# kerry-he/fsae-mpc

Measured on AMD Instinct MI355X. Metric: QP solves/sec (batched LTV-MPC, N=40 nx=5 nu=2 fp64), higher is better.
Workload: dtype f64

## Files before the change

### fsae-mpc_amd/csrc/qp_solver.hip

```cpp
#include <hip/hip_runtime.h>
#include <math.h>
#include <stdint.h>
#include <stdlib.h>
#include <stdio.h>
#include "qp_solver.h"

typedef double v4d __attribute__((ext_vector_type(4)));
typedef double v2d __attribute__((ext_vector_type(2)));

#define DEVINL __device__ __forceinline__
#ifndef QP_SOLVE_REFINE_STEPS
#define QP_SOLVE_REFINE_STEPS 1
#endif
#ifndef QP_FULL_BARRIERS
#define WAVE_SYNC() do { __builtin_amdgcn_fence(__ATOMIC_SEQ_CST, "wavefront"); __builtin_amdgcn_wave_barrier(); } while (0)
#else
#define WAVE_SYNC() __syncthreads()
#endif

namespace {

DEVINL double rl(double v, int src) {
  int lo = __builtin_amdgcn_readlane(__double2loint(v), src);
  int hi = __builtin_amdgcn_readlane(__double2hiint(v), src);
// ... 310 lines not shown
  for (int o = 1; o < NBIN; o <<= 1) {
    const int a = tid >= o ? scan[tid - o] : 0;
    __syncthreads();
    scan[tid] += a;
    __syncthreads();
  }
  int run = scan[tid] - v;
  for (int ww = 0; ww < NWV; ++ww) { const int c = cnt[ww][tid]; cnt[ww][tid] = run; run += c; }
  __syncthreads();
  if (w < NWV)
    for (int i0 = lo; i0 < hi; i0 += 512) {
      int kv[8];
#pragma unroll
      for (int r = 0; r < 8; ++r) { const int i = i0 + 64 * r + lane; kv[r] = i < hi ? bin(i) : -1; }
#pragma unroll
      for (int r = 0; r < 8; ++r) {
        const bool on = kv[r] >= 0; const int k = on ? kv[r] : 0;
        int rank, size; group(k, on, rank, size);
        int base = on ? cnt[w][k] : 0;
        if (on) order[base + rank] = i0 + 64 * r + lane;
        if (on && rank == 0) cnt[w][k] = base + size;
      }
    }
}

#endif

struct Ctx {
  int n, m, T, Kq, J, JB, JT, np, ld, lane, c, q, nc, nb, ntr;
  const int* perm; const int* tcs; const int* aoff; const int* tend;
  const double* Aw; const double* Hw; const double* Ab; const double* Hb;
  double* rows;
  double* ring;
  double* cof;
  int rowlen;
  double* Ms;
  double* vec;
};
enum VecArr { V_X = 0, V_G, V_HX, V_R1, V_R2, V_P1, V_P2, V_P3, V_DX, V_E, V_NARR };

DEVINL double* rowp(const Ctx& k, int arr) { return k.rows + (size_t)arr * k.rowlen; }
DEVINL double* vecp(const Ctx& k, int arr) { return k.vec + arr * k.np; }

DEVINL bool row_valid(const Ctx& k, int js) {
  if (js < k.J) { const int s = 16 * js + k.c; return s < k.Kq && 4 * s + k.q < k.m; }
  return (js - k.J) * 64 + k.lane < k.n;
}

template <int T> DEVINL void hx_tiles(const Ctx& k, const double* X, double* HX) {
  double hx[T], hn[T][4], hc[T][4];
#pragma unroll
  for (int t = 0; t < T; ++t) hx[t] = 0.0;
#pragma unroll
  for (int Jt = 0; Jt < T; ++Jt)
#pragma unroll
    for (int p = 0; p < 4; ++p) hn[Jt][p] = k.Hw[((size_t)Jt * 4 + p) * 64 + k.lane];
#pragma unroll 1
  for (int I = 0; I < T; ++I) {
#pragma unroll
    for (int Jt = 0; Jt < T; ++Jt)
#pragma unroll
      for (int p = 0; p < 4; ++p) hc[Jt][p] = hn[Jt][p];
    if (I + 1 < T) {
#pragma unroll
      for (int Jt = 0; Jt < T; ++Jt)
#pragma unroll
// ... 31 lines not shown
#pragma unroll
  for (int I = 0; I < T; ++I) {
    xc[I] = XV[16 * I + k.c]; sc[I] = 0.0;
#pragma unroll
    for (int p = 0; p < 4; ++p) { xr[I][p] = XV[16 * I + k.q + 4 * p]; sr[I][p] = 0.0; }
  }
#pragma unroll
  for (int I = 0; I < T; ++I)
#pragma unroll
    for (int J = I; J < T; ++J) {
      const v4d& h = acc[Tri<T>::idx(I, J)];
#pragma unroll
      for (int p = 0; p < 4; ++p) {
        sc[J] = fma(h[p], xr[I][p], sc[J]);
        if (J > I) sr[I][p] = fma(h[p], xc[J], sr[I][p]);
      }
    }
  WAVE_SYNC();
#pragma unroll
  for (int J = 0; J < T; ++J) { const double v = q_sum(sc[J]); if (k.q == 0) HX[16 * J + k.c] = v; }
  WAVE_SYNC();
#pragma unroll
  for (int I = 0; I < T - 1; ++I)
#pragma unroll
    for (int p = 0; p < 4; ++p) { const double v = grp16_sum(sr[I][p]); if (k.c == 0) HX[16 * I + k.q + 4 * p] += v; }
}

template <int C> struct IC { static constexpr int value = C; };

#ifdef QP_DRAIN_STREAM
template <int T> struct StreamCfg {
  static constexpr int R = 3 * T;
};
template <int T> struct Stream {
  static constexpr int R = StreamCfg<T>::R;
  const char* gnext;
  int half;
  DEVINL void issue(const Ctx& k, int slot) {
    __builtin_amdgcn_global_load_lds((const __attribute__((address_space(1))) void*)(gnext + k.lane * 16),
                                     (__attribute__((address_space(3))) void*)(k.ring + slot * 128), 16, 0, 0);
    gnext += 1024;
  }
  DEVINL void start(const Ctx& k, int c0) {
    gnext = reinterpret_cast<const char*>(k.Aw); half = 0;
#pragma unroll
    for (int t = 0; t < T; ++t) if (t < c0) issue(k, t);
  }
  template <int C> DEVINL void next_pair(const Ctx& k, v2d* b, int cn) {
    asm volatile("s_waitcnt vmcnt(0)" ::: "memory");
    const int other = (half ^ 1) * T;
#pragma unroll
    for (int t = 0; t < T; ++t) if (t < cn) issue(k, other + t);
    asm volatile("" ::: "memory");
#pragma unroll
    for (int t = 0; t < C; ++t) b[t] = *reinterpret_cast<const v2d*>(k.ring + (half * T + t) * 128 + k.lane * 2);
    half ^= 1;
  }
  DEVINL void drain() { asm volatile("s_waitcnt vmcnt(0)" ::: "memory"); }
};
#else
template <int T> struct StreamCfg {
  static constexpr int D = 2 * T;
  static constexpr int R = D + T;
};
template <int T> struct Stream {
  static constexpr int D = StreamCfg<T>::D, R = StreamCfg<T>::R;
  const char* gnext; int slot_i, slot_e;
  DEVINL void issue(const Ctx& k) {
    __builtin_amdgcn_global_load_lds((const __attribute__((address_space(1))) void*)(gnext + k.lane * 16),
                                     (__attribute__((address_space(3))) void*)(k.ring + slot_i * 128), 16, 0, 0);
    gnext += 1024;
    slot_i = slot_i + 1 == R ? 0 : slot_i + 1;
  }
  DEVINL void start(const Ctx& k, int) {
    gnext = reinterpret_cast<const char*>(k.Aw); slot_i = 0; slot_e = 0;
#pragma unroll
    for (int j = 0; j < D; ++j) issue(k);
  }
  template <int C> DEVINL void next_pair(const Ctx& k, v2d* b, int) {
#pragma unroll
    for (int t = 0; t < C; ++t) issue(k);
    asm volatile("s_waitcnt vmcnt(%0)" :: "n"(D) : "memory");
#pragma unroll
    for (int t = 0; t < C; ++t) {
      int sl = slot_e + t; if (sl >= R) sl -= R;
      b[t] = *reinterpret_cast<const v2d*>(k.ring + sl * 128 + k.lane * 2);
    }
    slot_e += C; if (slot_e >= R) slot_e -= R;
  }
  DEVINL void drain() { asm volatile("s_waitcnt vmcnt(0)" ::: "memory"); }
};
#endif

template <int NA> struct CoefStage {
  double reg[NA > 0 ? NA : 1];
  DEVINL void load(const Ctx& k, const double* const* arr, int js) {
    const int jc = js < k.J ? js : k.J - 1;
#pragma unroll
    for (int a = 0; a < NA; ++a) reg[a] = arr[a][jc * 64 + k.lane];
  }
  DEVINL void commit(const Ctx& k) {
#pragma unroll
    for (int a = 0; a < NA; ++a) k.cof[a * 64 + k.lane] = reg[a];
  }
  DEVINL void read_pair(const Ctx& k, int s, v2d* out) const {
#pragma unroll
    for (int a = 0; a < NA; ++a) out[a] = *reinterpret_cast<const v2d*>(k.cof + a * 64 + k.q * 16 + (s & 15));
  }
};

template <int T, int NB> DEVINL void pass_syrk(const Ctx& k, v4d* acc, double* P1, double* P2, double* P3, double* MB) {
  constexpr int NBB = NB > 0 ? NB : 1;
  constexpr int NA = 4 + NB;
  const int JS = k.J * 64;
  const double* arr[NA];
  arr[0] = rowp(k, R_D); arr[1] = rowp(k, R_W1); arr[2] = rowp(k, R_W2); arr[3] = rowp(k, R_W3);
#pragma unroll
  for (int e = 0; e < NB; ++e) arr[4 + e] = k.Ab + (size_t)e * JS;
  double p1[T], p2[T], p3[T];
  double pb[NBB][T], sbb[NBB][NBB], pwb[3][NBB];
#pragma unroll
  for (int t = 0; t < T; ++t) { p1[t] = 0; p2[t] = 0; p3[t] = 0; }
#pragma unroll
  for (int e = 0; e < NBB; ++e) {
#pragma unroll
    for (int t = 0; t < T; ++t) pb[e][t] = 0;
#pragma unroll
    for (int f = 0; f < NBB; ++f) sbb[e][f] = 0;
    pwb[0][e] = pwb[1][e] = pwb[2][e] = 0;
  }
  Stream<T> st;
  CoefStage<NA> cs;
  int tr = 0;
  if (k.ntr > 0) { st.start(k, k.tcs[0]); cs.load(k, arr, 0); }
  auto phase = [&](auto Cc) __attribute__((always_inline)) {
    constexpr int C = decltype(Cc)::value;
    const int tr_end = k.tend[C];
    for (; tr < tr_end; ++tr) {
      if ((tr & 3) == 0) { cs.commit(k); cs.load(k, arr, (tr >> 2) + 1); }
#pragma unroll
      for (int u = 0; u < 2; ++u) {
        v2d b[C], cf[NA];
        st.template next_pair<C>(k, b, u == 0 ? C : (tr + 1 < tr_end ? C : (tr + 1 < k.ntr ? k.tcs[tr + 1] : 0)));
        cs.read_pair(k, 4 * tr + 2 * u, cf);
        asm volatile("" ::: "memory");
#pragma unroll
        for (int h = 0; h < 2; ++h) {
          double a[C], ab[NBB];
          const double dd = cf[0][h], w1 = cf[1][h], w2 = cf[2][h], w3 = cf[3][h];
#pragma unroll
          for (int e = 0; e < NB; ++e) ab[e] = cf[4 + e][h];
#pragma unroll
          for (int t = 0; t < C; ++t) a[t] = dd * b[t][h];
#pragma unroll
          for (int I = 0; I < C; ++I)
#pragma unroll
            for (int Jt = I; Jt < C; ++Jt)
              acc[Tri<T>::idx(I, Jt)] = __builtin_amdgcn_mfma_f64_16x16x4f64(a[I], b[Jt][h], acc[Tri<T>::idx(I, Jt)], 0, 0, 0);
#pragma unroll
          for (int t = 0; t < C; ++t) {
            p1[t] = fma(w1, b[t][h], p1[t]); p2[t] = fma(w2, b[t][h], p2[t]); p3[t] = fma(w3, b[t][h], p3[t]);
          }
#pragma unroll
          for (int e = 0; e < NB; ++e) {
// ... 6 lines not shown
          }
        }
      }
    }
  };
  if constexpr (T >= 1) phase(IC<1>{});
  if constexpr (T >= 2) phase(IC<2>{});
  if constexpr (T >= 3) phase(IC<3>{});
  if constexpr (T >= 4) phase(IC<4>{});
  if constexpr (T >= 5) phase(IC<5>{});
  if constexpr (T >= 6) phase(IC<6>{});
  if constexpr (T >= 7) phase(IC<7>{});
  if constexpr (T >= 8) phase(IC<8>{});
  if (k.ntr > 0) st.drain();
#pragma unroll
  for (int t = 0; t < T; ++t) {
    double v1 = q_sum(p1[t]), v2 = q_sum(p2[t]), v3 = q_sum(p3[t]);
    if (k.q == 0) { P1[16 * t + k.c] = v1; P2[16 * t + k.c] = v2; P3[16 * t + k.c] = v3; }
  }
#pragma unroll
  for (int e = 0; e < NB; ++e) {
#pragma unroll
    for (int t = 0; t < T; ++t) { const double vb = q_sum(pb[e][t]); if (k.q == 0) MB[e * k.np + 16 * t + k.c] = vb; }
    const double v1 = q_sum(pwb[0][e]), v2 = q_sum(pwb[1][e]), v3 = q_sum(pwb[2][e]);
    if (k.lane == 0) { P1[k.nc + e] = v1; P2[k.nc + e] = v2; P3[k.nc + e] = v3; }
#pragma unroll
    for (int f = 0; f < NB; ++f) {
      const double sv = q_sum(f >= e ? sbb[e][f] : sbb[f][e]);
      if (k.lane == 0) MB[e * k.np + k.nc + f] = sv;
    }
  }
}

template <int T, int NB, int NVEC, int FUSE> DEVINL void pass_Av(const Ctx& k, const double* const* vin, double* const* rout, double* Pcor, double* Pcor2 = nullptr, const double* const* cfarr = nullptr) {
  constexpr int NBB = NB > 0 ? NB : 1;
  constexpr int NC = FUSE == 1 ? 6 : (FUSE >= 2 ? 3 : 0);
  constexpr int NA = NC + NB;
  const int JS = k.J * 64;
  const double* arr[NA > 0 ? NA : 1];
  if (FUSE == 1) { arr[0] = rowp(k, R_RPL); arr[1] = rowp(k, R_CB1); arr[2] = rowp(k, R_CC1); arr[3] = rowp(k, R_RPU); arr[4] = rowp(k, R_CB2); arr[5] = rowp(k, R_CC2); }
  if (FUSE >= 2) { arr[0] = cfarr ? cfarr[0] : rowp(k, R_CB1); arr[1] = cfarr ? cfarr[1] : rowp(k, R_RPL); arr[2] = cfarr ? cfarr[2] : rowp(k, R_CC1); }
#pragma unroll
  for (int f = 0; f < NB; ++f) arr[NC + f] = k.Ab + (size_t)f * JS;
  double v[NVEC][T], vb[NVEC][NBB], pc[T], pcb[NBB], pd[FUSE >= 2 ? T : 1], pdb[NBB];
#pragma unroll
  for (int e = 0; e < NVEC; ++e) {
#pragma unroll
    for (int t = 0; t < T; ++t) v[e][t] = vin[e][16 * t + k.c];
#pragma unroll
    for (int f = 0; f < NB; ++f) vb[e][f] = vin[e][k.nc + f];
  }
#pragma unroll
  for (int t = 0; t < T; ++t) pc[t] = 0.0;
#pragma unroll
  for (int f = 0; f < NBB; ++f) { pcb[f] = 0.0; pdb[f] = 0.0; }
#pragma unroll
  for (int t = 0; t < (FUSE >= 2 ? T : 1); ++t) pd[t] = 0.0;
  double keep[NVEC + 1];
#pragma unroll
  for (int e = 0; e < NVEC + 1; ++e) keep[e] = 0.0;
  Stream<T> st;
  CoefStage<NA> cs;
  int tr = 0;
  if (k.ntr > 0) { st.start(k, k.tcs[0]); if (NA > 0) cs.load(k, arr, 0); }
  auto phase = [&](auto Cc) __attribute__((always_inline)) {
    constexpr int C = decltype(Cc)::value;
    const int tr_end = k.tend[C];
    for (; tr < tr_end; ++tr) {
      if (NA > 0 && (tr & 3) == 0) { cs.commit(k); cs.load(k, arr, (tr >> 2) + 1); }
#pragma unroll
      for (int u = 0; u < 2; ++u) {
        v2d b[C], cf[NA > 0 ? NA : 1];
        st.template next_pair<C>(k, b, u == 0 ? C : (tr + 1 < tr_end ? C : (tr + 1 < k.ntr ? k.tcs[tr + 1] : 0)));
        if (NA > 0) cs.read_pair(k, 4 * tr + 2 * u, cf);
        asm volatile("" ::: "memory");
#pragma unroll
        for (int h = 0; h < 2; ++h) {
          const int s = 4 * tr + 2 * u + h;
          const int cc = s & 15;
#pragma unroll
          for (int e = 0; e < NVEC; ++e) {
            double dsum = 0.0;
#pragma unroll
            for (int t = 0; t < C; ++t) dsum = fma(b[t][h], v[e][t], dsum);
            dsum = grp16_sum(dsum);
#pragma unroll
            for (int f = 0; f < NB; ++f) dsum = fma(cf[NC + f][h], vb[e][f], dsum);
            if (k.c == cc) keep[e] = dsum;
            if (FUSE >= 2 && e == 0) {
              const double pen = cf[0][h] * (dsum - cf[1][h]);
              const double ynew = cf[2][h] - pen;
              if (k.c == cc) keep[NVEC] = ynew;
#pragma unroll
              for (int t = 0; t < C; ++t) { pc[t] = fma(ynew, b[t][h], pc[t]); pd[t] = fma(pen, b[t][h], pd[t]); }
// ... 300 lines not shown
      rh[K][p] = v;
    }
}
template <int T, int NS> DEVINL void rhs_store(const Ctx& k, const v4d* rh, double* const* vecs) {
#pragma unroll
  for (int K = 0; K < T; ++K)
#pragma unroll
    for (int p = 0; p < 4; ++p) {
      const int i = 16 * K + k.q + 4 * p;
#pragma unroll
      for (int e = 0; e < NS; ++e) if (k.c == e) vecs[e][i] = rh[K][p];
    }
}

#ifndef QP_STAMPS
#define QP_STAMPS 0
#endif
#if QP_STAMPS
#define STAMP_DECL unsigned long long st_acc[16]; for (int i_ = 0; i_ < 16; ++i_) st_acc[i_] = 0; unsigned long long st_t0 = __builtin_amdgcn_s_memtime();
#define STAMP(id) do { __builtin_amdgcn_sched_barrier(0); unsigned long long t_ = __builtin_amdgcn_s_memtime(); st_acc[id] += t_ - st_t0; st_t0 = t_; __builtin_amdgcn_sched_barrier(0); } while (0)
#define STAMP_OUT do { if (P.dump && P.dump_stage == 9 && lane == 0) for (int i_ = 0; i_ < 16; ++i_) P.dump[(size_t)b * 16 + i_] = (double)st_acc[i_]; } while (0)
#else
#define STAMP_DECL
#define STAMP(id) do { } while (0)
#define STAMP_OUT do { } while (0)
#endif

#ifndef QP_REFINE_ATTEMPTS
#define QP_REFINE_ATTEMPTS 3
#endif
#ifndef QP_WAVES_PER_SIMD
#define QP_WAVES_PER_SIMD 1
#endif
template <int T, int NB> __global__ __launch_bounds__(64, QP_WAVES_PER_SIMD) void qp_solve_kernel(QpParams P) {
  const int b = P.order ? P.order[blockIdx.x] : blockIdx.x;
  Ctx k;
  const QpDims& d = P.d;
  k.n = d.n; k.m = d.m; k.T = T; k.Kq = d.Kq; k.J = d.J; k.JB = d.JB; k.JT = d.J + d.JB; k.np = d.np; k.ld = 0;
  k.lane = threadIdx.x; k.c = k.lane & 15; k.q = k.lane >> 4; k.nc = d.nc; k.nb = d.nb;
  double* ws = P.ws + (size_t)b * d.ws_per_qp;
  k.Aw = ws + d.off_Aw; k.Hw = ws + d.off_Hw; k.Ab = ws + d.off_Ab; k.Hb = ws + d.off_Hb;
  k.rows = ws + d.off_rows; k.rowlen = d.rowlen; k.ntr = d.ntr;
  k.perm = reinterpret_cast<const int*>(ws + d.off_meta); k.tcs = k.perm + (size_t)(d.J > 0 ? d.J : 1) * 64;
  k.aoff = k.tcs + d.ntr; k.tend = k.aoff + d.ntr + 1;
  extern __shared__ double lds[];
  k.Ms = nullptr; k.vec = lds;
  double* MB = lds + (size_t)V_NARR * d.np;
  double* YL = MB + (size_t)(NB > 0 ? NB : 1) * d.np;
  k.ring = YL + T * 272;
  k.cof = k.ring + StreamCfg<T>::R * 128;
  double* SCR = k.ring;
  const double* gw = ws + d.off_gw;
  const double* Es = ws + d.off_E;
  const double* Fs = ws + d.off_F;
  const int lane = k.lane, n = k.n, JT = k.JT, J = k.J, nc = k.nc, nb = k.nb;
  constexpr int NT = Tri<T>::NT;
  constexpr int NBB = NB > 0 ? NB : 1;

#define X vecp(k, V_X)
#define G vecp(k, V_G)
#define HX vecp(k, V_HX)
#define R1 vecp(k, V_R1)
#define R2 vecp(k, V_R2)
#define P1 vecp(k, V_P1)
#define P2 vecp(k, V_P2)
#define P3 vecp(k, V_P3)
#define DX vecp(k, V_DX)
#define EV vecp(k, V_E)
#define aL rowp(k, R_L)
#define aU rowp(k, R_U)
#define aTL rowp(k, R_TL)
#define aTU rowp(k, R_TU)
#define aZL rowp(k, R_ZL)
#define aZU rowp(k, R_ZU)
#define aV rowp(k, R_V)
#define aD rowp(k, R_D)
#define aW1 rowp(k, R_W1)
#define aW2 rowp(k, R_W2)
#define aW3 rowp(k, R_W3)
#define aVA rowp(k, R_VA)
#define aVC rowp(k, R_VC)
#define aRPL rowp(k, R_RPL)
// ... 28 lines not shown
    double l = aL[ix], u = aU[ix];
    if (valid) {
      if (l > -INFINITY && u < INFINITY) {
        if (l > u) infeas = 1;
        if (!(u > l)) {
          const double eps = 1e-9 * fmax(1.0, fabs(l));
          l -= eps; u += eps; aL[ix] = l; aU[ix] = u;
        }
      }
      cnt_local += (l > -INFINITY) + (u < INFINITY);
    }
    if (js >= J) {
      const int i = (js - J) * 64 + lane;
      if (i < k.np) {
        double xi = 0.0;
        if (P.x_init) { const int ui = i < k.n ? qp_user_index(d, i) : -1; if (ui >= 0) { const double xs = P.x_init[(size_t)b * d.nu + ui] / EV[i]; if (fabs(xs) < INFINITY) xi = xs; } }
        if (valid) { if (l > -INFINITY && xi < l) xi = l; if (u < INFINITY && xi > u) xi = u; }
        X[i] = xi;
      }
    }
  }
  const double cnt = fmax(1.0, wave_sum((double)cnt_local));
  infeas = wave_max((double)infeas) > 0;
  WAVE_SYNC();

  STAMP_DECL
  int flag = 1, it = 0, flag_polished = 0;
  double fval_s = 0.0, merit_s = INFINITY;
  if (infeas) { flag = -2; }
  if (ws[d.off_bad] != 0.0) flag = -1;

  {
    const double* vin[1] = {X}; double* rout[1] = {aV};
    pass_Av<T, NB, 1, 0>(k, vin, rout, nullptr);
    for (int jb = 0; jb < k.JB; ++jb) { const int i = jb * 64 + lane; aV[(J + jb) * 64 + lane] = i < n ? X[i] : 0.0; }
  }
  const double T0 = 10.0, Z0 = 100.0;
  for (int js = 0; js < JT; ++js) {
    const int ix = js * 64 + lane;
    const bool valid = row_valid(k, js);
    const double l = aL[ix], u = aU[ix], v = aV[ix];
    const bool hl = valid && l > -INFINITY, hu = valid && u < INFINITY;
    aTL[ix] = hl ? fmax(v - l, T0) : 1.0;
    aTU[ix] = hu ? fmax(u - v, T0) : 1.0;
    aZL[ix] = hl ? Z0 : 0.0;
    aZU[ix] = hu ? Z0 : 0.0;
    aW3[ix] = (js < J) ? ((hl ? Z0 : 0.0) - (hu ? Z0 : 0.0)) : 0.0;
  }
  WAVE_SYNC();
  {
    hx_full(X);
    pass_Atw<T, NB>(k, aW3, P3);
    WAVE_SYNC();
    for (int jb = 0; jb < k.JB; ++jb) {
      const int i = jb * 64 + lane, ix = (J + jb) * 64 + lane;
      if (i < n) {
        const double r = HX[i] + G[i] - P3[i];
        if (aL[ix] > -INFINITY) aZL[ix] = fmax(r, 0.0) + Z0;
        if (aU[ix] < INFINITY) aZU[ix] = fmax(-r, 0.0) + Z0;
      }
    }
    WAVE_SYNC();
  }

  double saved_merit = INFINITY, best_res = INFINITY;
  int have_saved = 0, stall = 0;
  double* XS = ws + d.off_save;
  double* LAMS = ws + d.off_save + k.np;

  auto row1_body = [&](int ix, bool valid, double l, double u, double v, double tl, double tu, double zl, double zu,
                       double& s_gap, double& m_rp) {
    const bool hl = valid && l > -INFINITY, hu = valid && u < INFINITY;
    const double rpl = hl ? v - l - tl : 0.0, rpu = hu ? u - v - tu : 0.0;
    const double dl_ = hl ? zl / tl : 0.0, du_ = hu ? zu / tu : 0.0;
    aRPL[ix] = rpl; aRPU[ix] = rpu;
    rowp(k, R_CB1)[ix] = dl_; rowp(k, R_CC1)[ix] = hl ? dl_ / tl : 0.0;
    rowp(k, R_CB2)[ix] = du_; rowp(k, R_CC2)[ix] = hu ? du_ / tu : 0.0;
    aD[ix] = dl_ + du_;
    aW1[ix] = -dl_ * rpl + du_ * rpu;
    aW2[ix] = (hl ? 1.0 / tl : 0.0) - (hu ? 1.0 / tu : 0.0);
    aW3[ix] = (hl ? zl : 0.0) - (hu ? zu : 0.0);
    s_gap += (hl ? tl * zl : 0.0) + (hu ? tu * zu : 0.0);
    const double sc = fmax(1.0, fabs(v));
    if (hl) m_rp = fmax(m_rp, fabs(rpl) / fmax(sc, fabs(l)));
    if (hu) m_rp = fmax(m_rp, fabs(rpu) / fmax(sc, fabs(u)));
  };
  struct Slot { int ix; bool valid; double l, u, v, tl, tu, zl, zu, va, vc, w2, rpl, rpu; };
  auto load_slot = [&](int js) {
    Slot s_;
    const int jc = js < JT ? js : JT - 1;
    s_.ix = jc * 64 + lane; s_.valid = js < JT && row_valid(k, jc);
    const int ix = s_.ix;
    s_.l = aL[ix]; s_.u = aU[ix]; s_.v = aV[ix]; s_.tl = aTL[ix]; s_.tu = aTU[ix]; s_.zl = aZL[ix]; s_.zu = aZU[ix];
    s_.va = aVA[ix]; s_.vc = aVC[ix]; s_.w2 = aW2[ix]; s_.rpl = aRPL[ix]; s_.rpu = aRPU[ix];
    return s_;
  };
  double gap = 0.0, rp_rel = 0.0;

  v4d acc[NT];
  v4d rh[T];
  double Ubb[NBB][NBB];
  auto border_solve = [&](double* R) __attribute__((always_inline)) {
    if (NB > 0) {
      double yb[NBB], xb[NBB];
#pragma unroll
      for (int e = 0; e < NB; ++e) {
        double dsum = 0.0;
        for (int h = 0; h < 2; ++h) { const int i = lane + 64 * h; if (i < nc) dsum = fma(MB[e * k.np + i], R[i], dsum); }
        double tt = R[nc + e] - wave_sum(dsum);
#pragma unroll
        for (int g2 = 0; g2 < e; ++g2) tt -= Ubb[g2][e] * yb[g2];
        yb[e] = tt / Ubb[e][e];
      }
#pragma unroll
      for (int e = NB - 1; e >= 0; --e) {
        double tt = yb[e];
#pragma unroll
        for (int f = e + 1; f < NB; ++f) tt -= Ubb[e][f] * xb[f];
        xb[e] = tt / Ubb[e][e];
      }
      WAVE_SYNC();
      for (int h = 0; h < 2; ++h) {
        const int i = lane + 64 * h;
        if (i < nc) {
          double r = R[i];
#pragma unroll
          for (int e = 0; e < NB; ++e) r = fma(-MB[e * k.np + i], xb[e], r);
          R[i] = r;
// ... 132 lines not shown
  };
  auto solve1 = [&](double* V) __attribute__((always_inline)) {
#ifdef QP_MFMA_SOLVES
    const double* vin[1] = {V}; double* vout[1] = {V};
    rhs_load<T, 1>(k, rh, vin);
    reg_forward<T>(k, acc, YL, rh);
    if (NB > 0) {
      rhs_store<T, 1>(k, rh, vout);
      WAVE_SYNC();
      border_solve(V);
      rhs_load<T, 1>(k, rh, vin);
    }
    reg_backward<T>(k, acc, YL, rh, SCR);
    rhs_store<T, 1>(k, rh, vout);
#else
    double yv[T][4];
    vec_forward<T, false>(k, acc, YL, V, yv);
    if (NB > 0) {
      WAVE_SYNC();
      vec_rows_store<T>(k, yv, V);
      WAVE_SYNC();
      border_solve(V);
      vec_rows_load<T>(k, V, yv);
    }
    WAVE_SYNC();
    vec_backward<T, false>(k, acc, YL, yv, V);
#endif
  };

  STAMP(0);
  for (it = 0; flag == 1; ++it) {
    if (it == 0) {
      double s_gap = 0, m_rp = 0;
      for (int js = 0; js < JT; ++js) {
        const int ix = js * 64 + lane;
        row1_body(ix, row_valid(k, js), aL[ix], aU[ix], aV[ix], aTL[ix], aTU[ix], aZL[ix], aZU[ix], s_gap, m_rp);
      }
      gap = wave_sum(s_gap);
      rp_rel = wave_max(m_rp);
      WAVE_SYNC();
    }
    const double mu = gap / cnt;

    STAMP(1);
#ifdef QP_HX_SEPARATE
    hx_full(X);
    STAMP(2);
    acc_init<T>(k, acc);
#else
    acc_init<T>(k, acc);
    hx_from_acc<T>(k, acc, X, HX);
    hx_border(X);
    STAMP(2);
#endif
    pass_syrk<T, NB>(k, acc, P1, P2, P3, MB);
    WAVE_SYNC();
    STAMP(3);
    double fl = 0, m_rd = 0;
    for (int h = 0; h < 2; ++h) {
      const int i = lane + 64 * h;
      if (i < n) {
        const int ix = (J + (i >> 6)) * 64 + (i & 63);
        const double gz = P3[i] + aW3[ix];
        fl += 0.5 * X[i] * HX[i] + G[i] * X[i];
        const double sc = fmax(1.0, fmax(fabs(G[i]), fmax(fabs(HX[i]), fabs(gz))));
        m_rd = fmax(m_rd, fabs(HX[i] + G[i] - gz) / sc);
      }
    }
    const double fval = wave_sum(fl);
    const double rd_rel = wave_max(m_rd);
    const double gap_rel = gap / fmax(1.0, fabs(fval));
    const double merit = (fabs(fval) < INFINITY && fabs(gap_rel) < INFINITY) ? fmax(rd_rel, fmax(rp_rel, gap_rel)) : INFINITY;
    fval_s = fval; merit_s = merit;
    const bool res_ok = merit <= P.tol;
#ifdef QP_DEBUG_DUMP
    if (P.dump && P.dump_stage == 5 && b == P.dump_iter && lane == 0 && it < 120) {
      double* o_ = P.dump + 16 * it;
      o_[0] = merit; o_[1] = rd_rel; o_[2] = rp_rel; o_[3] = gap_rel; o_[4] = mu; o_[5] = fval; o_[6] = (double)have_saved; o_[7] = saved_merit;
    }
#endif
    if (!(merit < INFINITY)) { flag = have_saved ? 2 : -1; break; }
    if (merit <= P.tol_loose && merit < saved_merit) {
      for (int i = lane; i < k.np; i += 64) XS[i] = X[i];
      for (int js = 0; js < JT; ++js) LAMS[js * 64 + lane] = aW3[js * 64 + lane];
      have_saved = 1; saved_merit = merit;
    } else if (merit > P.tol_loose && rp_rel <= P.tol_loose && gap_rel <= P.tol_loose) {
      double dgap = 0, m_rd2 = 0, lamfix[2] = {0.0, 0.0};
      for (int h = 0; h < 2; ++h) {
// ... 53 lines not shown
    }
    if (it >= P.max_iter) { flag = have_saved ? 2 : 1; break; }

    {
      const double* vin[2] = {R1, R2}; double* rout[2] = {aVA, aVC};
      pass_Av<T, NB, 2, 1>(k, vin, rout, P1);
      for (int jb = 0; jb < k.JB; ++jb) {
        const int i = jb * 64 + lane;
        aVA[(J + jb) * 64 + lane] = i < n ? R1[i] : 0.0;
        aVC[(J + jb) * 64 + lane] = i < n ? R2[i] : 0.0;
      }
    }
    STAMP(7);
    double a_aff = 1.0, s1 = 0.0, s2 = 0.0;
    auto row2_body = [&](const Slot& r, int js) {
      const bool hl = r.valid && r.l > -INFINITY, hu = r.valid && r.u < INFINITY;
      double w = 0.0;
      if (hl) {
        const double dt = r.va + r.rpl, dz = -r.zl - (r.zl / r.tl) * dt;
        if (dt < 0) a_aff = fmin(a_aff, -r.tl / dt);
        if (dz < 0) a_aff = fmin(a_aff, -r.zl / dz);
        s1 += r.tl * dz + r.zl * dt; s2 += dt * dz;
        w -= dt * dz / r.tl;
      }
      if (hu) {
        const double dt = -r.va + r.rpu, dz = -r.zu - (r.zu / r.tu) * dt;
        if (dt < 0) a_aff = fmin(a_aff, -r.tu / dt);
        if (dz < 0) a_aff = fmin(a_aff, -r.zu / dz);
        s1 += r.tu * dz + r.zu * dt; s2 += dt * dz;
        w += dt * dz / r.tu;
      }
      if (js >= J && js < JT) aW1[r.ix] = w;
    };
    for (int js = 0; js < JT; js += 2) {
      const Slot r0 = load_slot(js), r1 = load_slot(js + 1);
      row2_body(r0, js); row2_body(r1, js + 1);
    }
    a_aff = wave_min(a_aff);
    s1 = wave_sum(s1); s2 = wave_sum(s2);
    const double mu_aff = fmax(0.0, gap + a_aff * (s1 + a_aff * s2)) / cnt;
    double sigma = mu > 0 ? (mu_aff / mu) * (mu_aff / mu) * (mu_aff / mu) : 0.0;
    if (sigma > 1.0) sigma = 1.0;
    {
      const double mu_floor = 1e-5 * P.tol * fmax(1.0, fabs(fval)) / cnt;
      if (mu > 0 && sigma < mu_floor / mu) sigma = fmin(1.0, mu_floor / mu);
    }
    const double smu = sigma * mu;
    const double cw = a_aff >= 0.05 ? 1.0 : 0.0;
    WAVE_SYNC();
    STAMP(8);
    if (cw != 0.0) {
    STAMP(9);
    for (int h = 0; h < 2; ++h) {
      const int i = lane + 64 * h;
      if (i < k.np) { const int ix = (J + (i >> 6)) * 64 + (i & 63); DX[i] = i < n ? P1[i] + aW1[ix] : 0.0; }
    }
    WAVE_SYNC();
    solve1(DX);
    WAVE_SYNC();
    STAMP(10);
    {
      const double* vin[1] = {DX}; double* rout[1] = {aW2};
      pass_Av<T, NB, 1, 0>(k, vin, rout, nullptr);
      for (int jb = 0; jb < k.JB; ++jb) { const int i = jb * 64 + lane; aW2[(J + jb) * 64 + lane] = i < n ? DX[i] : 0.0; }
    }
    STAMP(11);
    } else {
      for (int i = lane; i < k.np; i += 64) DX[i] = 0.0;
      for (int js = 0; js < JT; ++js) aW2[js * 64 + lane] = 0.0;
      WAVE_SYNC();
    }
    for (int h = 0; h < 2; ++h) {
      const int i = lane + 64 * h;
      if (i < n) DX[i] = R1[i] + smu * R2[i] + DX[i];
    }
    double amax = 1e300, bp = 0, bdp = 0, bd = 0, bdd = 0, q1 = 0.0, q2 = 0.0;
    auto row3a_body = [&](const Slot& r, int js) {
      const bool hl = r.valid && r.l > -INFINITY, hu = r.valid && r.u < INFINITY;
      const double dv = r.va + smu * r.vc + r.w2;
      if (js < JT) aVC[r.ix] = dv;
      if (hl) {
        const double dta = r.va + r.rpl, dza = -r.zl - (r.zl / r.tl) * dta;
        const double cl = smu - cw * dta * dza;
        const double dt = dv + r.rpl, dz = -r.zl + cl / r.tl - (r.zl / r.tl) * dt;
        if (dt < 0 && -r.tl / dt < amax) { amax = -r.tl / dt; bp = r.tl; bdp = dt; bd = r.zl; bdd = dz; }
        if (dz < 0 && -r.zl / dz < amax) { amax = -r.zl / dz; bp = r.zl; bdp = dz; bd = r.tl; bdd = dt; }
        q1 += r.tl * dz + r.zl * dt; q2 += dt * dz;
      }
      if (hu) {
        const double dta = -r.va + r.rpu, dza = -r.zu - (r.zu / r.tu) * dta;
        const double cu = smu - cw * dta * dza;
        const double dt = -dv + r.rpu, dz = -r.zu + cu / r.tu - (r.zu / r.tu) * dt;
        if (dt < 0 && -r.tu / dt < amax) { amax = -r.tu / dt; bp = r.tu; bdp = dt; bd = r.zu; bdd = dz; }
        if (dz < 0 && -r.zu / dz < amax) { amax = -r.zu / dz; bp = r.zu; bdp = dz; bd = r.tu; bdd = dt; }
        q1 += r.tu * dz + r.zu * dt; q2 += dt * dz;
      }
    };
    for (int js = 0; js < JT; js += 2) {
      const Slot r0 = load_slot(js), r1 = load_slot(js + 1);
      row3a_body(r0, js); row3a_body(r1, js + 1);
    }
    const double amax_w = wave_min(amax);
    double alpha = 1.0;
    if (amax_w < 1e299) {
      const unsigned long long msk = __ballot(amax == amax_w);
      const int src = __ffsll((long long)msk) - 1;
      bp = rl(bp, src); bdp = rl(bdp, src); bd = rl(bd, src); bdd = rl(bdd, src);
      q1 = wave_sum(q1); q2 = wave_sum(q2);
      const double gamma_f = 0.99, gamma_a = 1.0 / (1.0 - gamma_f);
      const double mufull = fmax(0.0, gap + amax_w * (q1 + amax_w * q2)) / cnt / gamma_a;
      const double a_h = (-bp + mufull / (bd + amax_w * bdd)) / bdp;
      alpha = fmin(1.0, fmin(0.99999999 * amax_w, fmax(a_h, gamma_f * amax_w)));
    }
#ifdef QP_DEBUG_DUMP
    if (P.dump && P.dump_stage == 5 && b == P.dump_iter && lane == 0 && it < 120) {
      double* o_ = P.dump + 16 * it;
      o_[8] = a_aff; o_[9] = sigma; o_[10] = alpha; o_[11] = cw; o_[12] = amax_w; o_[13] = (double)stall;
    }
    if (P.dump && b == 0 && P.dump_stage == 4 && it == P.dump_iter) {
      double c1 = 0, c2 = 0, c3 = 0, c4 = 0;
      for (int js = 0; js < JT; ++js) { const int ix = js * 64 + lane; c1 += aVA[ix]; c2 += aVC[ix]; c3 += aW2[ix]; c4 += aW1[ix]; }
      c1 = wave_sum(c1); c2 = wave_sum(c2); c3 = wave_sum(c3); c4 = wave_sum(c4);
      if (lane == 0) {
        double* o_ = P.dump;
        o_[0] = a_aff; o_[1] = mu_aff; o_[2] = sigma; o_[3] = smu; o_[4] = cw; o_[5] = amax_w; o_[6] = alpha; o_[7] = gap; o_[8] = mu;
        o_[9] = c1; o_[10] = c2; o_[11] = c3; o_[12] = c4; o_[13] = s1; o_[14] = s2; o_[15] = q1; o_[16] = q2;
      }
      for (int i = lane; i < n; i += 64) { P.dump[32 + i] = DX[i]; P.dump[32 + n + i] = R1[i]; P.dump[32 + 2 * n + i] = R2[i]; P.dump[32 + 3 * n + i] = P1[i]; }
    }
#endif
    double xn = 0, zn = 0, s_gap = 0, m_rp = 0;
    auto row3b_body = [&](const Slot& r, int js) {
      if (js >= JT) return;
      const bool hl = r.valid && r.l > -INFINITY, hu = r.valid && r.u < INFINITY;
      const double dv = r.vc;
      double tl = r.tl, zl = r.zl, tu = r.tu, zu = r.zu;
      if (hl) {
        const double dta = r.va + r.rpl, dza = -zl - (zl / tl) * dta;
        const double cl = smu - cw * dta * dza;
        const double dt = dv + r.rpl, dz = -zl + cl / tl - (zl / tl) * dt;
        tl += alpha * dt; zl += alpha * dz;
        aTL[r.ix] = tl; aZL[r.ix] = zl;
        zn = fmax(zn, zl);
      }
      if (hu) {
        const double dta = -r.va + r.rpu, dza = -zu - (zu / tu) * dta;
        const double cu = smu - cw * dta * dza;
        const double dt = -dv + r.rpu, dz = -zu + cu / tu - (zu / tu) * dt;
        tu += alpha * dt; zu += alpha * dz;
        aTU[r.ix] = tu; aZU[r.ix] = zu;
        zn = fmax(zn, zu);
      }
      const double v = r.v + alpha * dv;
      aV[r.ix] = v;
      row1_body(r.ix, r.valid, r.l, r.u, v, tl, tu, zl, zu, s_gap, m_rp);
    };
    for (int js = 0; js < JT; js += 2) {
      const Slot r0 = load_slot(js), r1 = load_slot(js + 1);
      row3b_body(r0, js); row3b_body(r1, js + 1);
    }
    for (int h = 0; h < 2; ++h) {
      const int i = lane + 64 * h;
      if (i < n) { X[i] += alpha * DX[i]; xn = fmax(xn, fabs(X[i])); }
    }
    const double rp_prev = rp_rel;
    gap = wave_sum(s_gap);
    rp_rel = wave_max(m_rp);
    xn = wave_max(xn); zn = wave_max(zn);
    WAVE_SYNC();
    STAMP(12);
    if (xn > 1e13) { flag = rp_prev > 1e-6 ? -2 : (fval < -1e13 ? -3 : -1); break; }
    if (zn > 1e15 && rp_prev > 1e-6) { flag = -2; break; }
    if (stall > (have_saved ? 5 : 25)) { flag = have_saved ? 2 : (rp_prev > 1e-6 ? -2 : (P.polish ? 5 : 1)); break; }
  }

  const bool v_current = flag == 0 || flag == 4;
  if (flag == 2) {
    for (int i = lane; i < k.np; i += 64) X[i] = XS[i];
    for (int js = 0; js < JT; ++js) aW3[js * 64 + lane] = LAMS[js * 64 + lane];
    flag = 0; merit_s = saved_merit;
    WAVE_SYNC();
  } else {
    for (int js = 0; js < JT; ++js) {
      const int ix = js * 64 + lane;
      const bool valid = row_valid(k, js);
      const bool hl = valid && aL[ix] > -INFINITY, hu = valid && aU[ix] < INFINITY;
      aW3[ix] = (hl ? aZL[ix] : 0.0) - (hu ? aZU[ix] : 0.0);
    }
    WAVE_SYNC();
  }
#ifdef QP_DEBUG_DUMP
  if (P.dump && P.dump_stage == 5 && b == P.dump_iter && lane == 0) { double* o_ = P.dump + 16 * 120; o_[4] = (double)flag; for (int i_ = 5; i_ < 48; ++i_) o_[i_] = 0.0; }
#endif
  if ((flag == 0 || flag == 4 || flag == 5) && P.polish) {
    const double rho = 1e6, pin = 1e16, rinv = 1.0 / rho;
    double* PA = rowp(k, R_CB1); double* PB = rowp(k, R_RPL); double* PY = rowp(k, R_CC1); double* PS = rowp(k, R_CB2);
    double* PC = rowp(k, R_RPU); double* PP = rowp(k, R_CC2); double* PZ0 = aW2;
    double* ATR = R1; double* ATP = P3;
    if (!v_current) {
      const double* vin[1] = {X}; double* rout[1] = {aV};
      pass_Av<T, NB, 1, 0>(k, vin, rout, nullptr);
      for (int jb = 0; jb < k.JB; ++jb) { const int i = jb * 64 + lane; aV[(J + jb) * 64 + lane] = i < n ? X[i] : 0.0; }
    }
    for (int js = 0; js < JT; ++js) {
      const int ix = js * 64 + lane;
      const bool valid = row_valid(k, js);
      const double l = aL[ix], u = aU[ix], v = aV[ix], lam = aW3[ix];
      const bool lo = valid && l > -INFINITY && lam > 0 && lam > fabs(v - l);
      const bool up = valid && u < INFINITY && lam < 0 && -lam > fabs(u - v);
      PS[ix] = lo ? 1.0 : (up ? -1.0 : 0.0); PY[ix] = ((lo || up) && js < J) ? lam : 0.0;
    }
    for (int i = lane; i < k.np; i += 64) XS[i] = X[i];
    WAVE_SYNC();
    for (int attempt = 0; attempt < QP_REFINE_ATTEMPTS && flag_polished <= 0; ++attempt) {
    for (int js = 0; js < JT; ++js) {
      const int ix = js * 64 + lane;
      const double sd = PS[ix];
      PA[ix] = sd != 0.0 ? rho : 0.0; PB[ix] = sd > 0 ? aL[ix] : (sd < 0 ? aU[ix] : 0.0);
      aD[ix] = js < J ? PA[ix] : (sd != 0.0 ? pin : 0.0); aW1[ix] = 0.0; aW2[ix] = 0.0; PC[ix] = 0.0; PP[ix] = 0.0;
    }
    WAVE_SYNC();
    acc_init<T>(k, acc);
    pass_syrk<T, NB>(k, acc, P1, P2, P3, MB);
    WAVE_SYNC();
    for (int i = lane; i < k.np; i += 64) { R1[i] = 0.0; R2[i] = 0.0; }
    WAVE_SYNC();
    bool pok = factor_solve2(-1) == 0, retry = false;
    if (!pok) { flag_polished = -5; break; }
    for (int h = 0; h < 2; ++h) {
      const int i = lane + 64 * h;
      if (i < k.np) { const int ix = (J + (i >> 6)) * 64 + (i & 63); R2[i] = (i < n && PS[ix] != 0.0) ? PB[ix] : XS[i]; }
    }
    WAVE_SYNC();
    const double* cf_eval[3] = {PA, PB, PY};
    const double* cf_cg[3] = {PA, PZ0, PZ0};
    auto eval_zy = [&]() __attribute__((always_inline)) {
      const double* vin[1] = {R2}; double* rout[2] = {aVA, aVC};
      pass_Av<T, NB, 1, 3>(k, vin, rout, P1, P2, cf_eval);
      hx_full(R2);
      WAVE_SYNC();
    };
    if (pok) {
      eval_zy();
      for (int h = 0; h < 2; ++h) {
        const int i = lane + 64 * h;
        if (i < k.np) { const int ix = (J + (i >> 6)) * 64 + (i & 63); DX[i] = (i < n && PS[ix] == 0.0) ? -(HX[i] + G[i] - P1[i]) : 0.0; }
      }
      WAVE_SYNC();
      solve1(DX);
      WAVE_SYNC();
      for (int h = 0; h < 2; ++h) {
        const int i = lane + 64 * h;
        if (i < n) { const int ix = (J + (i >> 6)) * 64 + (i & 63); if (PS[ix] == 0.0) R2[i] += DX[i]; }
      }
      WAVE_SYNC();
      eval_zy();
// ... 230 lines not shown
#undef DX
#undef EV
#if QP_MAIN_TU
__global__ void mfma_selftest_kernel(const double* Am, const double* Bm, double* Cm) {
  const int lane = threadIdx.x;
  const double a = Am[(lane & 15) * 4 + (lane >> 4)];
  const double bb = Bm[(lane >> 4) * 16 + (lane & 15)];
  v4d c = {0, 0, 0, 0};
  c = __builtin_amdgcn_mfma_f64_16x16x4f64(a, bb, c, 0, 0, 0);
#pragma unroll
  for (int p = 0; p < 4; ++p) Cm[((lane >> 4) + 4 * p) * 16 + (lane & 15)] = c[p];
}
#endif

}

#if QP_MAIN_TU

#ifdef QP_PROBE
template <int T, int NB> __global__ __launch_bounds__(64) void syrk_probe_kernel(QpParams P, int reps) {
  const int b = blockIdx.x;
  Ctx k;
  const QpDims& d = P.d;
  k.n = d.n; k.m = d.m; k.T = T; k.Kq = d.Kq; k.J = d.J; k.JB = d.JB; k.JT = d.J + d.JB; k.np = d.np; k.ld = 0;
  k.lane = threadIdx.x; k.c = k.lane & 15; k.q = k.lane >> 4; k.nc = d.nc; k.nb = d.nb;
  double* ws = P.ws + (size_t)b * d.ws_per_qp;
  k.Aw = ws + d.off_Aw; k.Hw = ws + d.off_Hw; k.Ab = ws + d.off_Ab; k.Hb = ws + d.off_Hb;
  k.rows = ws + d.off_rows; k.rowlen = d.rowlen; k.ntr = d.ntr;
  k.perm = reinterpret_cast<const int*>(ws + d.off_meta); k.tcs = k.perm + (size_t)(d.J > 0 ? d.J : 1) * 64;
  k.aoff = k.tcs + d.ntr; k.tend = k.aoff + d.ntr + 1;
  extern __shared__ double lds[];
  k.Ms = nullptr; k.vec = lds;
  double* MB = lds + (size_t)V_NARR * d.np;
  k.ring = MB + (size_t)(NB > 0 ? NB : 1) * d.np + T * 272; k.cof = k.ring + StreamCfg<T>::R * 128;
  for (int js = 0; js < k.JT; ++js) {
    const int ix = js * 64 + k.lane;
    rowp(k, R_D)[ix] = 1.0; rowp(k, R_W1)[ix] = 0.5; rowp(k, R_W2)[ix] = 0.25; rowp(k, R_W3)[ix] = 2.0;
  }
  __syncthreads();
  v4d acc[Tri<T>::NT];
  acc_init<T>(k, acc);
  const unsigned long long t0 = __builtin_amdgcn_s_memtime();
  for (int r = 0; r < reps; ++r) {
    pass_syrk<T, NB>(k, acc, vecp(k, V_P1), vecp(k, V_P2), vecp(k, V_P3), MB);
    __syncthreads();
  }
  const unsigned long long t1 = __builtin_amdgcn_s_memtime();
  double cs = 0;
#pragma unroll
  for (int i = 0; i < Tri<T>::NT; ++i) cs += acc[i][0] + acc[i][1] + acc[i][2] + acc[i][3];
  cs = wave_sum(cs);
  if (k.lane == 0) { P.dump[b] = (double)(t1 - t0) / reps; P.dump[gridDim.x + b] = cs; }
}
#endif

#ifdef QP_PROBE
template <int T> __global__ __launch_bounds__(64) void factor_probe_kernel(QpParams P, int reps) {
  const int b = blockIdx.x;
  Ctx k;
  const QpDims& d = P.d;
  k.n = d.n; k.m = d.m; k.T = T; k.Kq = d.Kq; k.J = d.J; k.JB = d.JB; k.JT = d.J + d.JB; k.np = d.np; k.ld = 0;
  k.lane = threadIdx.x; k.c = k.lane & 15; k.q = k.lane >> 4; k.nc = d.nc; k.nb = d.nb;
  double* ws = P.ws + (size_t)b * d.ws_per_qp;
  k.Aw = ws + d.off_Aw; k.Hw = ws + d.off_Hw; k.Ab = ws + d.off_Ab; k.Hb = ws + d.off_Hb;
  k.rows = ws + d.off_rows; k.rowlen = d.rowlen; k.ntr = d.ntr;
  extern __shared__ double lds[];
  k.Ms = nullptr; k.vec = lds;
  double* MB = lds + (size_t)V_NARR * d.np;
  double* YL = MB + (size_t)1 * d.np;
  k.ring = YL + T * 272; k.cof = k.ring + StreamCfg<T>::R * 128;
  double* SCR = k.ring;
  v4d acc[Tri<T>::NT], rh[T];
  unsigned long long tt[4] = {0, 0, 0, 0};
  double cs = 0;
  for (int r = 0; r < reps; ++r) {
    acc_init<T>(k, acc);
#pragma unroll
    for (int K = 0; K < T; ++K) {
#pragma unroll
      for (int p = 0; p < 4; ++p) { if (k.q + 4 * p == k.c) acc[Tri<T>::idx(K, K)][p] += 20.0; rh[K][p] = 1.0 + k.c; }
    }
    __builtin_amdgcn_sched_barrier(0);
    unsigned long long t0 = __builtin_amdgcn_s_memtime();
    reg_factor<T>(k, acc, YL, rh, 1e-30);
    __builtin_amdgcn_sched_barrier(0);
    unsigned long long t1 = __builtin_amdgcn_s_memtime();
    tt[0] += t1 - t0;
    v4d Yk;
#pragma unroll
    for (int K = 0; K < T; ++K) {
#pragma unroll
      for (int p = 0; p < 4; ++p) { Yk[p] = (k.q + 4 * p == k.c) ? 1.0 : 0.0; if (k.q + 4 * p == k.c) acc[Tri<T>::idx(K, K)][p] += 30.0; }
      diag_factor(k, acc[Tri<T>::idx(K, K)], Yk, rh[K], 1e-30);
      cs += Yk[0];
    }
    __builtin_amdgcn_sched_barrier(0);
    unsigned long long t2 = __builtin_amdgcn_s_memtime();
    tt[1] += t2 - t1;
#pragma unroll
    for (int K = 0; K < T; ++K) { tile_store(k, YL + K * 272, acc[Tri<T>::idx(K, K)]); __syncthreads(); acc[Tri<T>::idx(K, K)] = tile_load_t(k, YL + K * 272); }
    __builtin_amdgcn_sched_barrier(0);
    unsigned long long t3 = __builtin_amdgcn_s_memtime();
    tt[2] += t3 - t2;
// ... 228 lines not shown
```

Baseline: 375,700.

## Deepen LDS prefetch ring into idle YL space and chunk row sweeps

```diff
diff --git a/fsae-mpc_amd/csrc/qp_solver.hip b/fsae-mpc_amd/csrc/qp_solver.hip
--- a/fsae-mpc_amd/csrc/qp_solver.hip
+++ b/fsae-mpc_amd/csrc/qp_solver.hip
@@ -366,6 +366,7 @@
   const double* Aw; const double* Hw; const double* Ab; const double* Hb;
   double* rows;
   double* ring;
+  double* ringd;
   double* cof;
   int rowlen;
   double* Ms;
@@ -463,7 +464,7 @@
 template <int T> struct StreamCfg {
   static constexpr int R = 3 * T;
 };
-template <int T> struct Stream {
+template <int T, bool DEEP = false> struct Stream {
   static constexpr int R = StreamCfg<T>::R;
   const char* gnext;
   int half;
@@ -493,29 +494,59 @@
 template <int T> struct StreamCfg {
   static constexpr int D = 2 * T;
   static constexpr int R = D + T;
+#ifdef QP_SHALLOW_RING
+  static constexpr int RD = R;
+#else
+  static constexpr int RD = R + (T * 272) / 128;
+#endif
 };
-template <int T> struct Stream {
-  static constexpr int D = StreamCfg<T>::D, R = StreamCfg<T>::R;
-  const char* gnext; int slot_i, slot_e;
+template <int T, bool DEEP = false> struct Stream {
+  static constexpr int R = DEEP ? StreamCfg<T>::RD : StreamCfg<T>::R, D = R - T;
+  static_assert(D <= 56, "the lead must stay clear of the 6-bit vmcnt counter");
+  const char* gnext; int slot_i, slot_e, left;
+  DEVINL double* base(const Ctx& k) const { return DEEP && StreamCfg<T>::RD != StreamCfg<T>::R ? k.ringd : k.ring; }
   DEVINL void issue(const Ctx& k) {
     __builtin_amdgcn_global_load_lds((const __attribute__((address_space(1))) void*)(gnext + k.lane * 16),
-                                     (__attribute__((address_space(3))) void*)(k.ring + slot_i * 128), 16, 0, 0);
+                                     (__attribute__((address_space(3))) void*)(base(k) + slot_i * 128), 16, 0, 0);
     gnext += 1024;
     slot_i = slot_i + 1 == R ? 0 : slot_i + 1;
   }
   DEVINL void start(const Ctx& k, int) {
     gnext = reinterpret_cast<const char*>(k.Aw); slot_i = 0; slot_e = 0;
+#ifdef QP_STREAM_OVERRUN
+    left = 0;
 #pragma unroll
     for (int j = 0; j < D; ++j) issue(k);
+#else
+    left = k.aoff[k.ntr];
+#pragma unroll
+    for (int j = 0; j < D; ++j) if (j < left) issue(k);
+    left = left > D ? left - D : 0;
+#endif
   }
   template <int C> DEVINL void next_pair(const Ctx& k, v2d* b, int) {
+#ifdef QP_STREAM_OVERRUN
 #pragma unroll
     for (int t = 0; t < C; ++t) issue(k);
     asm volatile("s_waitcnt vmcnt(%0)" :: "n"(D) : "memory");
+#else
+    if (left >= C) {
+#pragma unroll
+      for (int t = 0; t < C; ++t) issue(k);
+      left -= C;
+      asm volatile("s_waitcnt vmcnt(%0)" :: "n"(D) : "memory");
+    } else if (left >= 0) {
+#pragma unroll
+      for (int t = 0; t < C - 1; ++t) if (t < left) issue(k);
+      left = -1;
+      asm volatile("s_waitcnt vmcnt(0)" ::: "memory");
+    }
+    asm volatile("" ::: "memory");
+#endif
 #pragma unroll
     for (int t = 0; t < C; ++t) {
       int sl = slot_e + t; if (sl >= R) sl -= R;
-      b[t] = *reinterpret_cast<const v2d*>(k.ring + sl * 128 + k.lane * 2);
+      b[t] = *reinterpret_cast<const v2d*>(base(k) + sl * 128 + k.lane * 2);
     }
     slot_e += C; if (slot_e >= R) slot_e -= R;
   }
@@ -540,7 +571,7 @@
   }
 };
 
-template <int T, int NB> DEVINL void pass_syrk(const Ctx& k, v4d* acc, double* P1, double* P2, double* P3, double* MB) {
+template <int T, int NB, bool DEEP> DEVINL void pass_syrk(const Ctx& k, v4d* acc, double* P1, double* P2, double* P3, double* MB) {
   constexpr int NBB = NB > 0 ? NB : 1;
   constexpr int NA = 4 + NB;
   const int JS = k.J * 64;
@@ -560,7 +591,7 @@
     for (int f = 0; f < NBB; ++f) sbb[e][f] = 0;
     pwb[0][e] = pwb[1][e] = pwb[2][e] = 0;
   }
-  Stream<T> st;
+  Stream<T, DEEP> st;
   CoefStage<NA> cs;
   int tr = 0;
   if (k.ntr > 0) { st.start(k, k.tcs[0]); cs.load(k, arr, 0); }
@@ -633,7 +664,7 @@
   }
 }
 
-template <int T, int NB, int NVEC, int FUSE> DEVINL void pass_Av(const Ctx& k, const double* const* vin, double* const* rout, double* Pcor, double* Pcor2 = nullptr, const double* const* cfarr = nullptr) {
+template <int T, int NB, int NVEC, int FUSE, bool DEEP = false> DEVINL void pass_Av(const Ctx& k, const double* const* vin, double* const* rout, double* Pcor, double* Pcor2 = nullptr, const double* const* cfarr = nullptr) {
   constexpr int NBB = NB > 0 ? NB : 1;
   constexpr int NC = FUSE == 1 ? 6 : (FUSE >= 2 ? 3 : 0);
   constexpr int NA = NC + NB;
@@ -660,7 +691,7 @@
   double keep[NVEC + 1];
 #pragma unroll
   for (int e = 0; e < NVEC + 1; ++e) keep[e] = 0.0;
-  Stream<T> st;
+  Stream<T, DEEP> st;
   CoefStage<NA> cs;
   int tr = 0;
   if (k.ntr > 0) { st.start(k, k.tcs[0]); if (NA > 0) cs.load(k, arr, 0); }
@@ -1027,6 +1058,11 @@
 #ifndef QP_WAVES_PER_SIMD
 #define QP_WAVES_PER_SIMD 1
 #endif
+#ifdef QP_ROW_CHUNK
+template <int T, int NB> struct RowChunk { static constexpr int value = QP_ROW_CHUNK; };
+#else
+template <int T, int NB> struct RowChunk { static constexpr int value = (T == 4 && NB == 4) ? 2 : ((NB == 4 || T >= 7) ? 4 : 6); };
+#endif
 template <int T, int NB> __global__ __launch_bounds__(64, QP_WAVES_PER_SIMD) void qp_solve_kernel(QpParams P) {
   const int b = P.order ? P.order[blockIdx.x] : blockIdx.x;
   Ctx k;
@@ -1043,6 +1079,7 @@
   double* MB = lds + (size_t)V_NARR * d.np;
   double* YL = MB + (size_t)(NB > 0 ? NB : 1) * d.np;
   k.ring = YL + T * 272;
+  k.ringd = YL;
   k.cof = k.ring + StreamCfg<T>::R * 128;
   double* SCR = k.ring;
   const double* gw = ws + d.off_gw;
@@ -1137,7 +1174,7 @@
 
   {
     const double* vin[1] = {X}; double* rout[1] = {aV};
-    pass_Av<T, NB, 1, 0>(k, vin, rout, nullptr);
+    pass_Av<T, NB, 1, 0, true>(k, vin, rout, nullptr);
     for (int jb = 0; jb < k.JB; ++jb) { const int i = jb * 64 + lane; aV[(J + jb) * 64 + lane] = i < n ? X[i] : 0.0; }
   }
   const double T0 = 10.0, Z0 = 100.0;
@@ -1197,8 +1234,34 @@
     s_.ix = jc * 64 + lane; s_.valid = js < JT && row_valid(k, jc);
     const int ix = s_.ix;
     s_.l = aL[ix]; s_.u = aU[ix]; s_.v = aV[ix]; s_.tl = aTL[ix]; s_.tu = aTU[ix]; s_.zl = aZL[ix]; s_.zu = aZU[ix];
-    s_.va = aVA[ix]; s_.vc = aVC[ix]; s_.w2 = aW2[ix]; s_.rpl = aRPL[ix]; s_.rpu = aRPU[ix];
+    s_.va = aVA[ix]; s_.vc = aVC[ix]; s_.w2 = aW2[ix];
+    s_.rpl = s_.v - s_.l - s_.tl; s_.rpu = s_.u - s_.v - s_.tu;
     return s_;
+  };
+  auto sweep = [&](auto&& body) __attribute__((always_inline)) {
+    constexpr int CH = RowChunk<T, NB>::value;
+    if constexpr (CH == 0) {
+      for (int js = 0; js < JT; js += 2) {
+        const Slot r0 = load_slot(js), r1 = load_slot(js + 1);
+        body(r0, js); body(r1, js + 1);
+      }
+    } else {
+      int js = 0;
+      for (; js + CH <= JT; js += CH) {
+        Slot rr[CH];
+#pragma unroll
+        for (int i = 0; i < CH; ++i) rr[i] = load_slot(js + i);
+#pragma unroll
+        for (int i = 0; i < CH; ++i) body(rr[i], js + i);
+      }
+      if (js < JT) {
+        Slot rr[CH > 1 ? CH - 1 : 1];
+#pragma unroll
+        for (int i = 0; i < CH - 1; ++i) if (js + i < JT) rr[i] = load_slot(js + i);
+#pragma unroll
+        for (int i = 0; i < CH - 1; ++i) if (js + i < JT) body(rr[i], js + i);
+      }
+    }
   };
   double gap = 0.0, rp_rel = 0.0;
 
@@ -1397,10 +1460,7 @@
   for (it = 0; flag == 1; ++it) {
     if (it == 0) {
       double s_gap = 0, m_rp = 0;
-      for (int js = 0; js < JT; ++js) {
-        const int ix = js * 64 + lane;
-        row1_body(ix, row_valid(k, js), aL[ix], aU[ix], aV[ix], aTL[ix], aTU[ix], aZL[ix], aZU[ix], s_gap, m_rp);
-      }
+      sweep([&](const Slot& r, int) { row1_body(r.ix, r.valid, r.l, r.u, r.v, r.tl, r.tu, r.zl, r.zu, s_gap, m_rp); });
       gap = wave_sum(s_gap);
       rp_rel = wave_max(m_rp);
       WAVE_SYNC();
@@ -1418,7 +1478,7 @@
     hx_border(X);
     STAMP(2);
 #endif
-    pass_syrk<T, NB>(k, acc, P1, P2, P3, MB);
+    pass_syrk<T, NB, true>(k, acc, P1, P2, P3, MB);
     WAVE_SYNC();
     STAMP(3);
     double fl = 0, m_rd = 0;
@@ -1538,10 +1598,7 @@
       }
       if (js >= J && js < JT) aW1[r.ix] = w;
     };
-    for (int js = 0; js < JT; js += 2) {
-      const Slot r0 = load_slot(js), r1 = load_slot(js + 1);
-      row2_body(r0, js); row2_body(r1, js + 1);
-    }
+    sweep(row2_body);
     a_aff = wave_min(a_aff);
     s1 = wave_sum(s1); s2 = wave_sum(s2);
     const double mu_aff = fmax(0.0, gap + a_aff * (s1 + a_aff * s2)) / cnt;
@@ -1567,7 +1624,7 @@
     STAMP(10);
     {
       const double* vin[1] = {DX}; double* rout[1] = {aW2};
-      pass_Av<T, NB, 1, 0>(k, vin, rout, nullptr);
+      pass_Av<T, NB, 1, 0, true>(k, vin, rout, nullptr);
       for (int jb = 0; jb < k.JB; ++jb) { const int i = jb * 64 + lane; aW2[(J + jb) * 64 + lane] = i < n ? DX[i] : 0.0; }
     }
     STAMP(11);
@@ -1602,10 +1659,7 @@
         q1 += r.tu * dz + r.zu * dt; q2 += dt * dz;
       }
     };
-    for (int js = 0; js < JT; js += 2) {
-      const Slot r0 = load_slot(js), r1 = load_slot(js + 1);
-      row3a_body(r0, js); row3a_body(r1, js + 1);
-    }
+    sweep(row3a_body);
     const double amax_w = wave_min(amax);
     double alpha = 1.0;
     if (amax_w < 1e299) {
@@ -1661,10 +1715,7 @@
       aV[r.ix] = v;
       row1_body(r.ix, r.valid, r.l, r.u, v, tl, tu, zl, zu, s_gap, m_rp);
     };
-    for (int js = 0; js < JT; js += 2) {
-      const Slot r0 = load_slot(js), r1 = load_slot(js + 1);
-      row3b_body(r0, js); row3b_body(r1, js + 1);
-    }
+    sweep(row3b_body);
     for (int h = 0; h < 2; ++h) {
       const int i = lane + 64 * h;
       if (i < n) { X[i] += alpha * DX[i]; xn = fmax(xn, fabs(X[i])); }
@@ -1705,7 +1756,7 @@
     double* ATR = R1; double* ATP = P3;
     if (!v_current) {
       const double* vin[1] = {X}; double* rout[1] = {aV};
-      pass_Av<T, NB, 1, 0>(k, vin, rout, nullptr);
+      pass_Av<T, NB, 1, 0, true>(k, vin, rout, nullptr);
       for (int jb = 0; jb < k.JB; ++jb) { const int i = jb * 64 + lane; aV[(J + jb) * 64 + lane] = i < n ? X[i] : 0.0; }
     }
     for (int js = 0; js < JT; ++js) {
@@ -1727,7 +1778,7 @@
     }
     WAVE_SYNC();
     acc_init<T>(k, acc);
-    pass_syrk<T, NB>(k, acc, P1, P2, P3, MB);
+    pass_syrk<T, NB, true>(k, acc, P1, P2, P3, MB);
     WAVE_SYNC();
     for (int i = lane; i < k.np; i += 64) { R1[i] = 0.0; R2[i] = 0.0; }
     WAVE_SYNC();
@@ -2024,7 +2075,7 @@
   extern __shared__ double lds[];
   k.Ms = nullptr; k.vec = lds;
   double* MB = lds + (size_t)V_NARR * d.np;
-  k.ring = MB + (size_t)(NB > 0 ? NB : 1) * d.np + T * 272; k.cof = k.ring + StreamCfg<T>::R * 128;
+  k.ringd = MB + (size_t)(NB > 0 ? NB : 1) * d.np; k.ring = k.ringd + T * 272; k.cof = k.ring + StreamCfg<T>::R * 128;
   for (int js = 0; js < k.JT; ++js) {
     const int ix = js * 64 + k.lane;
     rowp(k, R_D)[ix] = 1.0; rowp(k, R_W1)[ix] = 0.5; rowp(k, R_W2)[ix] = 0.25; rowp(k, R_W3)[ix] = 2.0;
@@ -2034,7 +2085,7 @@
   acc_init<T>(k, acc);
   const unsigned long long t0 = __builtin_amdgcn_s_memtime();
   for (int r = 0; r < reps; ++r) {
-    pass_syrk<T, NB>(k, acc, vecp(k, V_P1), vecp(k, V_P2), vecp(k, V_P3), MB);
+    pass_syrk<T, NB, true>(k, acc, vecp(k, V_P1), vecp(k, V_P2), vecp(k, V_P3), MB);
     __syncthreads();
   }
   const unsigned long long t1 = __builtin_amdgcn_s_memtime();
@@ -2060,7 +2111,7 @@
   k.Ms = nullptr; k.vec = lds;
   double* MB = lds + (size_t)V_NARR * d.np;
   double* YL = MB + (size_t)1 * d.np;
-  k.ring = YL + T * 272; k.cof = k.ring + StreamCfg<T>::R * 128;
+  k.ring = YL + T * 272; k.ringd = YL; k.cof = k.ring + StreamCfg<T>::R * 128;
   double* SCR = k.ring;
   v4d acc[Tri<T>::NT], rh[T];
   unsigned long long tt[4] = {0, 0, 0, 0};
```

Result: slower. 363,600 (-3.2%).
